# sumansamui/CMOOP_Audio_Processing

Hardware: AMD Instinct MI355X
Metric: candidate-net evals/hour (pop=40, GSC-v2) (higher is better)
Workload: dtype f32

## Files before the change

### cmoop_audio_processing_amd/_lib.py

```python
from __future__ import annotations

import ctypes as C
import os
import re
import subprocess
import threading

_HERE = os.path.dirname(os.path.abspath(__file__))
CSRC = os.path.join(_HERE, "csrc")
LIB_PATH = os.environ.get("CMOOP_LIB_PATH") or os.path.join(CSRC, "libcmoop_hip.so")
HEADER = os.path.join(os.path.dirname(_HERE), "include", "cmoop.h")

_lock = threading.Lock()
_lib = None


class CmoopError(RuntimeError):
    pass


class Config(C.Structure):
    _fields_ = [(n, C.c_int32) for n in (
        "variant", "classes", "epochs", "batch", "patience", "early_stop", "restore_best", "acc_readout",
        "fpr_variant", "shuffle", "eval_batch", "n_slots", "profile_every", "gemm_mode")] + \
# ... 93 lines not shown
    "cmoop_bn_train_fwd": [_V] * 10 + [_I64, _I32, _F64, _F64, _I32, _I32],
    "cmoop_bn_eval_fwd": [_V] * 8 + [_I64, _I32, _F64, _I32],
    "cmoop_bn_bwd": [_V] * 9 + [_I64, _I32, _I32, _I32],
    "cmoop_bn_pool_fwd": [_V] * 5 + [_I32] * 5,
    "cmoop_bn_pool_bwd": [_V] * 10 + [_I32] * 6,
    "cmoop_add_relu": [_V, _V, _V, _I64],
    "cmoop_gap_fwd": [_V, _V, _I32, _I32, _I32],
    "cmoop_gap_bwd": [_V, _V, _V, _I32, _I32, _I32],
    "cmoop_softmax_ce": [_V, _V, _V, _I64, _I64, _I32, _I32, _V, _V, _V],
    "cmoop_softmax_probs": [_V, _V, _I32, _I32],
    "cmoop_adam": [_V, _V, _V, _V, _I64, _F64, _F64, _F64, _F64],
    "cmoop_adam_segments": [_V] * 5 + [_I32] + [_V] * 5 + [_F64] * 4,
    "cmoop_confusion": [_V, _V, _I64, _I32, _I32, _V],
    "cmoop_colsum_small": [_V, _V, _I32, _I32],
    "cmoop_dense_dgrad_small": [_V, _V, _V, _I32, _I32, _I32, _V, _F64],
}


_U32 = C.c_uint32
DENSE_PROTOTYPES = {
    "cmoop_dense_fwd_ex": [_V] * 4 + [_I32] * 5 + [_F64, _U32, _I32, _U32, _V],
    "cmoop_dense_bwd_ex": [_V] * 6 + [_I32] * 4 + [_F64, _I32, _I32],
}

DWCONV_PROTOTYPES = {
    "cmoop_dwconv_fwd": [_V] * 3 + [_I32] * 5,
    "cmoop_dwconv_bwd": [_V] * 5 + [_I32] * 6,
    "cmoop_dwconv_wgrad_slices": [_I32] * 5 + [_V],
    "cmoop_dwconv_time": [_I32] + [_V] * 4 + [_I32] * 6 + [_V],
    "cmoop_plan_dwconvs": [_V, _I32, _I32, _I32, _V, _I32, _V],
# ... 27 lines not shown
                f"{LIB_PATH} is missing: run `python -c 'import __graft_entry__ as g; g.build()'` "
                "(or `make -C cmoop_audio_processing_amd/csrc`). There is no CPU fallback for this path.")
        try:
            L = C.CDLL(LIB_PATH)
        except OSError as e:
            raise CmoopError(f"cannot load {LIB_PATH}: {e}") from e
        L.cmoop_last_error.restype = C.c_char_p
        L.cmoop_abi_version.restype = C.c_int
        for name in declared_symbols():
            fn = getattr(L, name)
            if name not in ("cmoop_last_error", "cmoop_config_default"):
                fn.restype = C.c_int
        L.cmoop_config_default.restype = None
        for name, argtypes in list(STREAM_PROTOTYPES.items()) + list(AUGMENT_PROTOTYPES.items()) + list(PCEN_PROTOTYPES.items()) + \
                list(ELEM_PROTOTYPES.items()) + list(LOSS_PROTOTYPES.items()) + list(DENSE_PROTOTYPES.items()) + list(DWCONV_PROTOTYPES.items()) + \
                list(DISTILL_PROTOTYPES.items()):
            getattr(L, name).argtypes = argtypes
        _lib = L
        return L


def check(rc: int) -> None:
    if rc != 0:
        raise CmoopError(lib().cmoop_last_error().decode("utf-8", "replace"))


def default_config() -> Config:
    c = Config()
    lib().cmoop_config_default(C.byref(c))
    return c

# ... 65 lines not shown
```

### cmoop_audio_processing_amd/csrc/api.hip

```cpp
#include "../../include/cmoop.h"
#include "net.h"

#include <cstring>
#include <memory>
#include <mutex>
#include <vector>

using namespace cmoop;

static thread_local std::string g_err;
static thread_local std::string g_last_kernels;

template <class F>
static int guard(F&& f) {
    try {
        f();
        return 0;
    } catch (const std::exception& e) {
        g_err = e.what();
        return 1;
    } catch (...) {
        g_err = "unknown error";
        return 2;
    }
// ... 881 lines not shown
        h->net->drain_profile();
    });
}
int cmoop_net_get_state(cmoop_net* h, float* params, float* adam_m, float* adam_v, int64_t* iterations, int64_t* steps) {
    return guard([&] {
        long long it = 0, st = 0;
        h->net->get_state(params, adam_m, adam_v, &it, &st);
        if (iterations) *iterations = it;
        if (steps) *steps = st;
    });
}
int cmoop_net_set_state(cmoop_net* h, const float* params, const float* adam_m, const float* adam_v, int64_t iterations,
                        int64_t steps) {
    return guard([&] { h->net->set_state(params, adam_m, adam_v, iterations, steps); });
}
int cmoop_net_set_augment(cmoop_net* h, const cmoop_augment* aug) {
    return guard([&] {
        CMOOP_REQUIRE(h && h->net, "set_augment: NULL net");
        if (!aug) { h->net->set_augment(nullptr); return; }
        const AugmentCfg c = to_augment(aug);
        h->net->set_augment(&c);
    });
}
int cmoop_net_set_loss(cmoop_net* h, const cmoop_loss* loss) {
    return guard([&] {
        CMOOP_REQUIRE(h && h->net, "set_loss: NULL net");
        if (!loss) { h->net->set_loss(nullptr); return; }
        const LossCfg c = to_loss(loss);
        h->net->set_loss(&c);
    });
// ... 461 lines not shown
int cmoop_bn_pool_bwd(const float* g_pooled, const uint8_t* arg, const float* x, const float* mean, const float* invstd,
                      const float* gamma, float* dx, float* dgamma, float* dbeta, float* sums, int32_t B, int32_t H, int32_t W,
                      int32_t C, int32_t mask_x_pos, int32_t blocks) {
    return guard([&] {
        CMOOP_REQUIRE(B >= 1 && H >= 1 && W >= 1, "bn_pool_bwd: empty tensor");
        const int nb = reduce_blocks_arg(blocks, (int64_t)B * H * W, C);
        hipStream_t s = lib_stream();
        Scratch ws(s);
        float* P = ws.floats((size_t)nb * 2 * C + 2 * C);
        launch_bn_pool_bwd_reduce(g_pooled, arg, x, mean, invstd, P, B, H, W, C, nb, s);
        launch_bn_pool_bwd_apply(g_pooled, arg, x, mean, invstd, gamma, P, nb, dx, dgamma, dbeta, B, H, W, C, mask_x_pos, s);
        if (sums) CMOOP_HIP(hipMemcpyAsync(sums, P + (size_t)nb * 2 * C, (size_t)2 * C * 4, hipMemcpyDeviceToDevice, s));
        CMOOP_HIP(hipStreamSynchronize(s));
    });
}
int cmoop_add_relu(const float* a, const float* b, float* y, int64_t n) {
    return guard([&] {
        hipStream_t s = lib_stream();
        launch_add_relu(a, b, y, n, s);
        CMOOP_HIP(hipStreamSynchronize(s));
    });
}
int cmoop_gap_fwd(const float* x, float* y, int32_t B, int32_t HW, int32_t C) {
    return guard([&] {
        CMOOP_REQUIRE(B >= 0 && HW >= 1 && C >= 4, "gap_fwd: HW >= 1, C >= 4");
        hipStream_t s = lib_stream();
        launch_gap_fwd(x, y, B, HW, C, s);
        CMOOP_HIP(hipStreamSynchronize(s));
    });
}
// ... 83 lines not shown
```

### cmoop_audio_processing_amd/csrc/elem.hip

```cpp
#include "kernels.h"
#include <cstdlib>
#include <algorithm>
#include <cmath>
#include <mutex>

namespace cmoop {

typedef float f32x4 __attribute__((ext_vector_type(4)));

__device__ __forceinline__ int64_t gather_row(const int32_t* __restrict__ idx, int64_t pos, int64_t n_rows) {
    int64_t src = idx ? (int64_t)idx[pos] : pos;
    if (n_rows > 0) src = src < 0 ? 0 : (src >= n_rows ? n_rows - 1 : src);
    return src;
}

template <int KS>
__global__ __launch_bounds__(256) void conv1_fwd_kernel(const float* __restrict__ X, const int32_t* __restrict__ idx,
                                                        int64_t row0, const float* __restrict__ Wt,
                                                        const float* __restrict__ bias, float* __restrict__ Y, int B,
                                                        int H, int W, int Cout, int relu, const StepState* __restrict__ st,
                                                        int64_t n_rows) {
    constexpr int TAPS = KS * KS, SEG = 4 + KS - 1, p = (KS - 1) >> 1;
    __shared__ __attribute__((aligned(16))) float Ws[TAPS * 64];
    if (st) row0 = st->row0;
// ... 704 lines not shown
    if (i >= M * K) return;
    const int m = i / K, k = i - m * K;
    float s = 0.f;
    for (int o = 0; o < N; ++o) s = fmaf(dY[(size_t)m * N + o], W[(size_t)o * K + k], s);
    if (mask) s = mask[i] > 0.f ? s * scale : 0.f;
    dX[i] = s;
}

void launch_dense_dgrad_small(const float* dY, const float* W, float* dX, int M, int N, int K, const float* mask,
                              float scale, hipStream_t s) {
    if (M * K == 0) return;
    hipLaunchKernelGGL(dense_dgrad_small_kernel, dim3(cdiv(M * K, 256)), dim3(256), 0, s, dY, W, dX, M, N, K, mask, scale);
    CMOOP_HIP(hipGetLastError());
}

__global__ __launch_bounds__(256) void maxpool_fwd_kernel(const float* __restrict__ X, float* __restrict__ Y,
                                                          uint8_t* __restrict__ arg, int B, int H, int W, int C, int OH,
                                                          int OW) {
    const int C4 = C >> 2;
    const int64_t n = (int64_t)B * OH * OW * C4;
    for (int64_t i = (int64_t)blockIdx.x * 256 + threadIdx.x; i < n; i += (int64_t)gridDim.x * 256) {
        const int c4 = (int)(i % C4);
        int64_t p = i / C4;
        const int ow = (int)(p % OW); p /= OW;
        const int oh = (int)(p % OH);
        const int b = (int)(p / OH);
        f32x4 best;
        uchar4 a = {0, 0, 0, 0};
        bool first = true;
#pragma unroll
        for (int pos = 0; pos < 4; ++pos) {
            const int ih = 2 * oh + (pos >> 1), iw = 2 * ow + (pos & 1);
            if (ih >= H || iw >= W) continue;
            const f32x4 v = *reinterpret_cast<const f32x4*>(X + ((size_t)(b * H + ih) * W + iw) * C + 4 * c4);
            if (first) { best = v; first = false; continue; }
            if (v[0] > best[0]) { best[0] = v[0]; a.x = pos; }
            if (v[1] > best[1]) { best[1] = v[1]; a.y = pos; }
            if (v[2] > best[2]) { best[2] = v[2]; a.z = pos; }
            if (v[3] > best[3]) { best[3] = v[3]; a.w = pos; }
        }
        *reinterpret_cast<f32x4*>(Y + i * 4) = best;
        *reinterpret_cast<uchar4*>(arg + i * 4) = a;
    }
}

void launch_maxpool_fwd(const float* X, float* Y, uint8_t* arg, int B, int H, int W, int C, hipStream_t s) {
    CMOOP_REQUIRE(C % 4 == 0, "maxpool: C % 4");
    const int OH = (H + 1) / 2, OW = (W + 1) / 2;
    const int64_t n = (int64_t)B * OH * OW * (C / 4);
    if (n == 0) return;
    hipLaunchKernelGGL(maxpool_fwd_kernel, dim3(ew_grid(n)), dim3(256), 0, s, X, Y, arg, B, H, W, C, OH, OW);
    CMOOP_HIP(hipGetLastError());
}

__global__ __launch_bounds__(256) void maxpool_bwd_kernel(const float* __restrict__ dY, const uint8_t* __restrict__ arg,
                                                          const float* __restrict__ Y, float* __restrict__ dX, int B,
                                                          int H, int W, int C, int OH, int OW, int mask_y_pos) {
    const int C4 = C >> 2;
    const int64_t n = (int64_t)B * OH * OW * C4;
    for (int64_t i = (int64_t)blockIdx.x * 256 + threadIdx.x; i < n; i += (int64_t)gridDim.x * 256) {
        const int c4 = (int)(i % C4);
        int64_t p = i / C4;
        const int ow = (int)(p % OW); p /= OW;
        const int oh = (int)(p % OH);
        const int b = (int)(p / OH);
        f32x4 g = *reinterpret_cast<const f32x4*>(dY + i * 4);
// ... 14 lines not shown
            *reinterpret_cast<f32x4*>(dX + ((size_t)(b * H + ih) * W + iw) * C + 4 * c4) = o;
        }
    }
}

void launch_maxpool_bwd(const float* dY, const uint8_t* arg, const float* Y, float* dX, int B, int H, int W, int C,
                        int mask_y_pos, hipStream_t s) {
    const int OH = (H + 1) / 2, OW = (W + 1) / 2;
    const int64_t n = (int64_t)B * OH * OW * (C / 4);
    if (n == 0) return;
    hipLaunchKernelGGL(maxpool_bwd_kernel, dim3(ew_grid(n)), dim3(256), 0, s, dY, arg, Y, dX, B, H, W, C, OH, OW,
                       mask_y_pos);
    CMOOP_HIP(hipGetLastError());
}

__global__ __launch_bounds__(256) void bn_pool_fwd_kernel(const float* __restrict__ X, float* __restrict__ Y,
                                                          uint8_t* __restrict__ arg, const float* __restrict__ scale,
                                                          const float* __restrict__ shift, int B, int H, int W, int C,
                                                          int OH, int OW, int relu) {
    const int C4 = C >> 2;
    const int64_t n = (int64_t)B * OH * OW * C4;
    for (int64_t i = (int64_t)blockIdx.x * 256 + threadIdx.x; i < n; i += (int64_t)gridDim.x * 256) {
        const int c4 = (int)(i % C4);
        int64_t p = i / C4;
        const int ow = (int)(p % OW); p /= OW;
        const int oh = (int)(p % OH);
        const int b = (int)(p / OH);
        const f32x4 sc = *reinterpret_cast<const f32x4*>(scale + 4 * c4);
        const f32x4 sh = *reinterpret_cast<const f32x4*>(shift + 4 * c4);
        f32x4 best;
        uchar4 a = {0, 0, 0, 0};
        bool first = true;
#pragma unroll
        for (int pos = 0; pos < 4; ++pos) {
            const int ih = 2 * oh + (pos >> 1), iw = 2 * ow + (pos & 1);
            if (ih >= H || iw >= W) continue;
            const f32x4 x = *reinterpret_cast<const f32x4*>(X + ((size_t)(b * H + ih) * W + iw) * C + 4 * c4);
            f32x4 v;
#pragma unroll
            for (int j = 0; j < 4; ++j) {
                const float t = x[j] * sc[j] + sh[j];
                v[j] = relu ? fmaxf(t, 0.f) : t;
            }
            if (first) { best = v; first = false; continue; }
            if (v[0] > best[0]) { best[0] = v[0]; a.x = pos; }
            if (v[1] > best[1]) { best[1] = v[1]; a.y = pos; }
            if (v[2] > best[2]) { best[2] = v[2]; a.z = pos; }
            if (v[3] > best[3]) { best[3] = v[3]; a.w = pos; }
        }
        *reinterpret_cast<f32x4*>(Y + i * 4) = best;
        *reinterpret_cast<uchar4*>(arg + i * 4) = a;
    }
}

void launch_bn_pool_fwd(const float* X, float* Y, uint8_t* arg, const float* scale, const float* shift, int B, int H, int W,
                        int C, int relu, hipStream_t s) {
    CMOOP_REQUIRE(C % 4 == 0, "bn_pool: C % 4");
    const int OH = (H + 1) / 2, OW = (W + 1) / 2;
    const int64_t n = (int64_t)B * OH * OW * (C / 4);
    if (n == 0) return;
    hipLaunchKernelGGL(bn_pool_fwd_kernel, dim3(ew_grid(n)), dim3(256), 0, s, X, Y, arg, scale, shift, B, H, W, C, OH, OW, relu);
    CMOOP_HIP(hipGetLastError());
}

struct PooledGrad {
    const float* g; const uint8_t* arg;
    int H, W, OH, OW, C;
    __device__ __forceinline__ f32x4 at(int64_t row, int c) const {
        const int iw = (int)(row % W);
        const int64_t t = row / W;
        const int ih = (int)(t % H), b = (int)(t / H);
        const size_t o = (((size_t)b * OH + (ih >> 1)) * OW + (iw >> 1)) * C + c;
        const f32x4 gv = *reinterpret_cast<const f32x4*>(g + o);
        const uchar4 a = *reinterpret_cast<const uchar4*>(arg + o);
        const int pos = ((ih & 1) << 1) | (iw & 1);
        return f32x4{a.x == pos ? gv[0] : 0.f, a.y == pos ? gv[1] : 0.f, a.z == pos ? gv[2] : 0.f, a.w == pos ? gv[3] : 0.f};
// ... 1033 lines not shown
```

### cmoop_audio_processing_amd/csrc/kernels.h

```cpp
#pragma once
#include "common.h"
#include <string>
#include <vector>

namespace cmoop {

struct ConvGeom {
    int B, H, W, Cin;
    int OH, OW, Cout;
    int KH, KW, stride;
    int pad_t, pad_l;
    int M() const { return B * OH * OW; }
    int K() const { return KH * KW * Cin; }
};
inline ConvGeom conv_geometry(int B, int H, int W, int Cin, int Cout, int KS, int stride) {
    ConvGeom g;
    g.B = B; g.H = H; g.W = W; g.Cin = Cin; g.Cout = Cout; g.KH = g.KW = KS; g.stride = stride;
    g.OH = (H + stride - 1) / stride; g.OW = (W + stride - 1) / stride;
    const int th = (g.OH - 1) * stride + KS - H, tw = (g.OW - 1) * stride + KS - W;
    g.pad_t = (th > 0 ? th : 0) / 2; g.pad_l = (tw > 0 ? tw : 0) / 2;
    return g;
}

enum GemmMode { GEMM_DEFAULT = -1, GEMM_FP32 = 0, GEMM_FP32_DMA = 1 , GEMM_BF16X3 = 2, GEMM_BF16 = 3,
// ... 177 lines not shown
void launch_bn_finalize(const float* P, int blocks, int64_t M, int C, const float* gamma, const float* beta,
                        float* moving_mean, float* moving_var, float* mean, float* invstd, float* scale,
                        float* shift, float eps, float momentum, float one_minus_momentum, hipStream_t s);
void launch_bn_eval_prepare(const float* gamma, const float* beta, const float* moving_mean,
                            const float* moving_var, float* scale, float* shift, int C, float eps, hipStream_t s);
void launch_scale_shift(const float* X, float* Y, const float* scale, const float* shift, int64_t M, int C,
                        int relu, hipStream_t s);
void launch_bn_bwd_apply(const float* dY, const float* X, const float* mean, const float* invstd,
                         const float* gamma, const float* P, int blocks, float* dX, float* dgamma, float* dbeta,
                         int64_t M, int C, int mask_x_pos, hipStream_t s);
void launch_colsum_small(const float* X, float* out, int M, int C, hipStream_t s);
void launch_dense_dgrad_small(const float* dY, const float* W, float* dX, int M, int N, int K, const float* mask,
                              float scale, hipStream_t s);
void launch_colsum_finalize(const float* P, int blocks, int C, float* out, hipStream_t s);

void launch_maxpool_fwd(const float* X, float* Y, uint8_t* arg, int B, int H, int W, int C, hipStream_t s);
void launch_maxpool_bwd(const float* dY, const uint8_t* arg, const float* Y, float* dX, int B, int H, int W, int C,
                        int mask_y_pos, hipStream_t s);
void launch_bn_pool_fwd(const float* X, float* Y, uint8_t* arg, const float* scale, const float* shift, int B, int H, int W,
                        int C, int relu, hipStream_t s);
void launch_bn_pool_bwd_reduce(const float* g_pooled, const uint8_t* arg, const float* X, const float* mean, const float* invstd,
                               float* P, int B, int H, int W, int C, int blocks, hipStream_t s);
void launch_bn_pool_bwd_apply(const float* g_pooled, const uint8_t* arg, const float* X, const float* mean, const float* invstd,
                              const float* gamma, const float* P, int blocks, float* dX, float* dgamma, float* dbeta, int B,
                              int H, int W, int C, int mask_x_pos, hipStream_t s);
void launch_add_relu(const float* A, const float* Bt, float* Y, int64_t n, hipStream_t s);
void launch_gap_fwd(const float* X, float* Y, int B, int HW, int C, hipStream_t s);
void launch_gap_bwd(const float* dY, const float* X, float* dX, int B, int HW, int C, hipStream_t s);
void launch_softmax_ce(const float* Z, const int32_t* labels, const int32_t* idx, int64_t row0, int B, int C,
                       float* dZ, double* acc, int32_t* preds, hipStream_t s, const StepState* st = nullptr, int64_t n_rows = 0);
void launch_softmax_probs(const float* Z, float* P, int B, int C, hipStream_t s);
void launch_window_gather(const float* feat, float* chunk, int64_t w0, int B, int hop, int T, int F, int db, int db_ref_max,
                          float amin, float top_db, const double* mean, const double* scale, hipStream_t s);
void launch_adam(float* w, const float* g, float* m, float* v, int64_t n, float alpha, float c1, float c2,
                 float eps, hipStream_t s, const StepState* st = nullptr, const float* alpha_table = nullptr);
// ... 65 lines not shown
```

### cmoop_audio_processing_amd/csrc/net.h

```cpp
#pragma once
#include "kernels.h"
#include <atomic>
#include <functional>
#include <map>
#include <mutex>
#include <set>
#include <string>
#include <vector>

namespace cmoop {

struct NetConfig {
    int variant = 0, classes = 10, epochs = 300, batch = 64, patience = 5;
    int early_stop = 1, restore_best = 0, acc_readout = 0, fpr_variant = 0, shuffle = 1;
    int eval_batch = 256, n_slots = 8, profile_every = 0;
    int gemm_mode = GEMM_FP32;
    double lr = 1e-3, beta1 = 0.9, beta2 = 0.999, adam_eps = 1e-7, bn_eps = 1e-3, bn_momentum = 0.99, dropout = 0.3;
};

struct DropoutParams {
    uint32_t thr;
    float keep_scale;
    static uint32_t stream(int layer) { return STREAM_DROPOUT + (uint32_t)layer; }
};
// ... 97 lines not shown
    int rowtab_rows = 0;
    void* rowtab_d = nullptr;
    int rowtab_d_rows = 0;
    int64_t w_off = 0, b_off = 0, wd_off = -1;
    int64_t slab_off = -1;
    size_t slab_floats = 0;
    int tensor_index = 0;
    int64_t gamma_off = 0, beta_off = 0, mm_off = 0, mv_off = 0;
    int relu_after = 0, mask_in_pos = 0;
    int fuse_pool = 0;
    int feeds_bn = 0;
    float* bn_buf = nullptr;
    uint8_t* arg = nullptr;
    int mask_y_pos = 0;
    int fused_into_bn = 0;
};

struct NetPlan {
    std::vector<Act> acts;
    std::vector<Op> ops;
    int logits = -1;
    int64_t n_params = 0;
    size_t splitk_floats(int batch, int Bmax) const;
    std::string launch_plan(int batch, int Bmax, int B, bool train) const;
};
NetPlan plan_net(const int32_t gene[6], const NetConfig& cfg, int T, int F);

class Net : public GemmHook {
  public:
    const GemmTiming* begin(int cls, double flops) override;
// ... 19 lines not shown
    void run_epoch(const float* X, const int32_t* y, int64_t n_train, int epoch, int32_t* idx_scratch);

    void train_step(const float* X, const int32_t* y, const int32_t* idx, int64_t row0, int B);
    void train_step_targets(const float* x_rows, const float* t, const float* w, const int32_t* primary, int B);
    void train_step_distill_targets(const float* x_rows, const float* t, const float* w, const int32_t* primary, const float* q,
                                    double alpha, double temperature, int B);
    void begin_fit(int64_t total_steps);
    void begin_epoch();
    void train_step_stateful(const float* X, const int32_t* y, const int32_t* idx, int B);
    void evaluate(const float* X, const int32_t* y, int64_t n, double* loss_sum, long long* correct, int32_t* preds);
    void predict(const float* X, int64_t n, float* probs);
    void predict_logits(const float* X, int64_t n, float* logits);
    void predict_stream(const float* feat, int64_t n_frames, int hop, bool db_scale, bool db_ref_max, float db_amin, float top_db,
                        const double* mean, const double* scale, float* probs);
    void read_train_metrics(double* loss_sum, long long* correct, bool reset);
    void drain_profile();
    hipStream_t stream() const { return stream_; }
    uint32_t seed() const { return seed_; }
    const NetConfig& config() const { return cfg_; }
    int feature_T() const { return T_; }
    int feature_F() const { return F_; }
    long long steps_done() const { return step_; }
    long long iterations_done() const { return iterations_; }

  private:
    void build_plan();
    void forward(const float* X, const int32_t* idx, int64_t row0, int B, bool train, const StepState* st = nullptr);
    void backward(const float* X, const int32_t* idx, int64_t row0, int B, const StepState* st = nullptr);
    void step_body(const float* X, const int32_t* y, const int32_t* idx, int64_t row0, int B, const StepState* st);
    void optimiser_step(int B, const StepState* st);
    ConvBuffers buffers_of(const Op& op) const;
    float* dalloc(size_t floats);

    int32_t gene_[6];
    NetConfig cfg_;
    int T_, F_, Bmax_;
    uint32_t seed_;
    hipStream_t stream_;
    std::vector<Act> acts_;
    std::vector<Op> ops_;
    std::vector<void*> allocs_;
    int64_t n_params_ = 0;
// ... 63 lines not shown
```

### cmoop_audio_processing_amd/csrc/net.hip

```cpp
#include "net.h"

#include <algorithm>
#include <chrono>
#include <cmath>
#include <cstdlib>
#include <cstring>
#include <functional>
#include <map>
#include <numeric>
#include <thread>

namespace cmoop {

static const int FC_LADDER[5][4] = {{0, 0, 0, 0}, {64, 0, 0, 0}, {128, 64, 0, 0}, {256, 128, 64, 0}, {512, 256, 128, 64}};

void validate_gene(const int32_t g[6]) {
    const bool ok = (g[0] == 16 || g[0] == 32 || g[0] == 64) && (g[1] == 3 || g[1] == 5) && (g[2] == 0 || g[2] == 1) &&
                    (g[3] >= 1 && g[3] <= 3) && (g[4] >= 1 && g[4] <= 4) && (g[5] == 0 || g[5] == 1);
    CMOOP_REQUIRE(ok, "gene outside the search space (filters{16,32,64}, kernel{3,5}, bn{0,1}, res{1..3}, fc{1..4}, dropout{0,1})");
}

DropoutParams dropout_params(double rate) {
    CMOOP_REQUIRE(rate >= 0.0 && rate < 1.0, "dropout must be in [0,1)");
    return DropoutParams{(uint32_t)(rate * 16777216.0), (float)(1.0 / (1.0 - rate))};
// ... 259 lines not shown
        const int skip = add_conv(OP_CONV, x, 2 * c, 1, 2, 0, in_relu, 1.f, 1);
        int y;
        if (A) {
            y = add_sepconv(x, 2 * c, k, !bn, in_relu);
            if (bn) y = add_bn(y, 1, 0);
            y = add_sepconv(y, 2 * c, k, 0, 1);
            if (bn) y = add_bn(y, 0, 0);
            y = add_pool(y, 0);
        } else {
            y = add_sepconv(x, 2 * c, k, 1, in_relu);
            if (bn) y = add_bn(y, 0, 1);
            y = add_pool(y, !bn);
        }
        Op op; op.kind = OP_ADDRELU; op.in = y; op.in2 = skip;
        op.out = new_act(acts[y].H, acts[y].W, acts[y].C);
        ops.push_back(op);
        x = op.out;
        c *= 2;
    }
    {
        Op op; op.kind = OP_GAP; op.in = x;
        op.out = new_act(1, 1, acts[x].C);
        ops.push_back(op);
        x = op.out;
    }
    const float keep_scale = dropout_params(cfg.dropout).keep_scale;
    for (int i = 0; i < fc; ++i) {
        const int in_relu = i > 0;
        const float ms = (in_relu && dr) ? keep_scale : 1.f;
        x = add_conv(OP_DENSE, x, FC_LADDER[fc][i], 1, 1, 1, in_relu, ms, 0);
// ... 402 lines not shown
        case OP_BN: {
            const Act& ia = acts_[op.in];
            const int64_t M = (int64_t)B * ia.H * ia.W;
            const int C = op.Cout;
            float *mean = op.bn_buf, *invstd = mean + C, *scale = invstd + C, *shift = scale + C;
            if (train) {
                int nb = fused_stats_blocks_;
                fused_stats_blocks_ = 0;
                if (nb == 0) {
                    nb = colreduce_blocks(M, C);
                    launch_colstats(ia.data, red_ws_, M, C, nb, stream_);
                }
                launch_bn_finalize(red_ws_, nb, M, C, params_ + op.gamma_off, params_ + op.beta_off, params_ + op.mm_off,
                                   params_ + op.mv_off, mean, invstd, scale, shift, (float)cfg_.bn_eps, (float)cfg_.bn_momentum,
                                   (float)(1.0 - cfg_.bn_momentum), stream_);
            } else {
                launch_bn_eval_prepare(params_ + op.gamma_off, params_ + op.beta_off, params_ + op.mm_off,
                                       params_ + op.mv_off, scale, shift, C, (float)cfg_.bn_eps, stream_);
            }
            if (op.fuse_pool) {
                const Op& pool = ops_[oi + 1];
                launch_bn_pool_fwd(ia.data, acts_[pool.out].data, pool.arg, scale, shift, B, ia.H, ia.W, C, op.relu_after, stream_);
            } else {
                launch_scale_shift(ia.data, acts_[op.out].data, scale, shift, M, C, op.relu_after, stream_);
            }
            break;
        }
        case OP_POOL: {
            if (op.fused_into_bn) break;
            const Act& ia = acts_[op.in];
            launch_maxpool_fwd(ia.data, acts_[op.out].data, op.arg, B, ia.H, ia.W, ia.C, stream_);
            break;
        }
        case OP_ADDRELU:
            launch_add_relu(acts_[op.in].data, acts_[op.in2].data, acts_[op.out].data,
                            (int64_t)B * acts_[op.out].per_sample(), stream_);
            break;
        case OP_GAP: {
            const Act& ia = acts_[op.in];
            launch_gap_fwd(ia.data, acts_[op.out].data, B, ia.H * ia.W, ia.C, stream_);
            break;
        }
        }
    }
}

void Net::backward(const float* X, const int32_t* idx, int64_t row0, int B, const StepState* st) {
    slab_segs_.clear();
    launch_flip_transpose_all(params_, wd_ws_, flip_table_, flip_layers_, flip_max_elems_, stream_);
    for (int oi = (int)ops_.size() - 1; oi >= 0; --oi) {
        const Op& op = ops_[oi];
        switch (op.kind) {
        case OP_DENSE: {
            const float* dY = acts_[op.out].grad;
            Act& ia = acts_[op.in];
            const char* du = std::getenv("CMOOP_DENSE_UNFUSED");
            const bool unfused = du && du[0] == '1';
            if (!unfused) {
                launch_dense_bwd(ia.data, dY, params_ + op.w_off, grads_ + op.w_off, grads_ + op.b_off, ia.grad, B, op.Cout, op.Cin,
// ... 41 lines not shown
            if (op.fuse_pool) {
                const Op& pool = ops_[oi + 1];
                launch_bn_pool_bwd_reduce(acts_[pool.out].grad, pool.arg, ia.data, mean, invstd, red_ws_, B, ia.H, ia.W, C, nb, stream_);
                launch_bn_pool_bwd_apply(acts_[pool.out].grad, pool.arg, ia.data, mean, invstd, params_ + op.gamma_off, red_ws_, nb,
                                         ia.grad, grads_ + op.gamma_off, grads_ + op.beta_off, B, ia.H, ia.W, C, op.mask_in_pos, stream_);
                break;
            }
            launch_bn_bwd_reduce(acts_[op.out].grad, ia.data, mean, invstd, red_ws_, M, C, nb, stream_);
            launch_bn_bwd_apply(acts_[op.out].grad, ia.data, mean, invstd, params_ + op.gamma_off, red_ws_, nb, ia.grad,
                                grads_ + op.gamma_off, grads_ + op.beta_off, M, C, op.mask_in_pos, stream_);
            break;
        }
        case OP_POOL: {
            if (op.fused_into_bn) break;
            const Act& ia = acts_[op.in];
            launch_maxpool_bwd(acts_[op.out].grad, op.arg, acts_[op.out].data, ia.grad, B, ia.H, ia.W, ia.C, op.mask_y_pos,
                               stream_);
            break;
        }
        case OP_ADDRELU:
            break;
        case OP_GAP: {
            const Act& ia = acts_[op.in];
            launch_gap_bwd(acts_[op.out].grad, ia.data, ia.grad, B, ia.H * ia.W, ia.C, stream_);
            break;
        }
        case OP_CONV1: {
            if (batch_in_)
                launch_conv1_wgrad(batch_in_, nullptr, 0, acts_[op.out].grad, wgrad_ws_ + op.slab_off, B, T_, F_, op.Cout, op.KS, stream_,
                                   nullptr, 0);
// ... 141 lines not shown
    std::vector<float> tab(total_steps);
    const double b1 = cfg_.beta1, b2 = cfg_.beta2;
    for (int64_t i = 0; i < total_steps; ++i) {
        const double t = (double)(i + 1);
        tab[i] = (float)(cfg_.lr * std::sqrt(1.0 - std::pow(b2, t)) / (1.0 - std::pow(b1, t)));
    }
    alpha_tab_ = dalloc(total_steps);
    alpha_tab_n_ = total_steps;
    if (!st_dev_) st_dev_ = reinterpret_cast<StepState*>(dalloc(8));
    CMOOP_HIP(hipMemcpyAsync(alpha_tab_, tab.data(), total_steps * 4, hipMemcpyHostToDevice, stream_));
    const StepState st0{0, (unsigned)step_, (unsigned)iterations_};
    CMOOP_HIP(hipMemcpyAsync(st_dev_, &st0, sizeof(StepState), hipMemcpyHostToDevice, stream_));
    CMOOP_HIP(hipStreamSynchronize(stream_));
    static const bool use_graph = [] { const char* v = std::getenv("CMOOP_GRAPH"); return v && v[0] == '1'; }();
    if (!use_graph) graph_ok_ = false;
}

void Net::begin_epoch() {
    host_row0_ = 0;
    if (st_dev_) CMOOP_HIP(hipMemsetAsync(&st_dev_->row0, 0, sizeof(long long), stream_));
}

void Net::train_step_stateful(const float* X, const int32_t* y, const int32_t* idx, int B) {
    CMOOP_REQUIRE(B >= 1 && B <= cfg_.batch, "train batch larger than configured");
    if (!st_dev_) {
        train_step(X, y, idx, host_row0_, B);
        host_row0_ += B;
        return;
    }
    CMOOP_REQUIRE(iterations_ < alpha_tab_n_, "train_step_stateful outside begin_fit's step budget");
// ... 164 lines not shown
        }
        idx = idx_scratch;
    }
    if (st_dev_) {
        const StepState st0{0, (unsigned)step_, (unsigned)iterations_};
        CMOOP_HIP(hipMemcpyAsync(st_dev_, &st0, sizeof(StepState), hipMemcpyHostToDevice, stream_));
        CMOOP_HIP(hipStreamSynchronize(stream_));
    }
    begin_epoch();
    for (int64_t s = 0; s < n_train; s += cfg_.batch)
        train_step_stateful(X, y, idx, (int)std::min<int64_t>(cfg_.batch, n_train - s));
}

void Net::evaluate(const float* X, const int32_t* y, int64_t n, double* loss_sum, long long* correct, int32_t* preds) {
    CMOOP_HIP(hipMemsetAsync(acc_eval_, 0, 16, stream_));
    for (int64_t s = 0; s < n; s += cfg_.eval_batch) {
        const int B = (int)std::min<int64_t>(cfg_.eval_batch, n - s);
        forward(X, nullptr, s, B, false);
        launch_softmax_ce(acts_[logits_].data, y, nullptr, s, B, cfg_.classes, nullptr, acc_eval_, preds ? preds + s : nullptr,
                          stream_);
    }
    double host[2];
    CMOOP_HIP(hipMemcpyAsync(host, acc_eval_, 16, hipMemcpyDeviceToHost, stream_));
    CMOOP_HIP(hipStreamSynchronize(stream_));
    *loss_sum = host[0];
    std::memcpy(correct, &host[1], 8);
}

void Net::predict(const float* X, int64_t n, float* probs) {
    CMOOP_REQUIRE(n >= 0 && (n == 0 || (X && probs)), "predict: NULL buffer");
    for (int64_t s = 0; s < n; s += cfg_.eval_batch) {
        const int B = (int)std::min<int64_t>(cfg_.eval_batch, n - s);
        forward(X, nullptr, s, B, false);
        launch_softmax_probs(acts_[logits_].data, probs + s * cfg_.classes, B, cfg_.classes, stream_);
    }
    CMOOP_HIP(hipStreamSynchronize(stream_));
}

void Net::predict_logits(const float* X, int64_t n, float* logits) {
    CMOOP_REQUIRE(n >= 0 && (n == 0 || (X && logits)), "predict_logits: NULL buffer");
    for (int64_t s = 0; s < n; s += cfg_.eval_batch) {
        const int B = (int)std::min<int64_t>(cfg_.eval_batch, n - s);
        forward(X, nullptr, s, B, false);
        CMOOP_HIP(hipMemcpyAsync(logits + s * cfg_.classes, acts_[logits_].data, (size_t)B * cfg_.classes * 4, hipMemcpyDeviceToDevice,
                                 stream_));
    }
    CMOOP_HIP(hipStreamSynchronize(stream_));
}

int64_t stream_windows(int64_t n_frames, int T, int hop) {
    CMOOP_REQUIRE(hop >= 1, "stream windows: hop_frames must be at least 1");
    CMOOP_REQUIRE(T >= 1 && n_frames >= T, "stream windows: the stream has " + std::to_string(n_frames) + " frames, a window needs " + std::to_string(T));
    return 1 + (n_frames - T) / hop;
}

void Net::predict_stream(const float* feat, int64_t n_frames, int hop, bool db_scale, bool db_ref_max, float db_amin, float top_db,
                         const double* mean, const double* scale, float* probs) {
    const int64_t n = stream_windows(n_frames, T_, hop);
    CMOOP_REQUIRE(feat && probs, "predict_stream: NULL buffer");
    CMOOP_REQUIRE((mean == nullptr) == (scale == nullptr), "predict_stream: mean and scale come together (both or neither)");
    const int B0 = (int)std::min<int64_t>(cfg_.eval_batch, n);
    float* chunk = static_cast<float*>(pool_alloc((size_t)B0 * T_ * F_ * 4));
    double* ms = mean ? static_cast<double*>(pool_alloc((size_t)2 * F_ * 8)) : nullptr;
    auto cleanup = [&]() { hipStreamSynchronize(stream_); pool_free(chunk); if (ms) pool_free(ms); };
    try {
        if (ms) {
            CMOOP_HIP(hipMemcpyAsync(ms, mean, (size_t)F_ * 8, hipMemcpyHostToDevice, stream_));
            CMOOP_HIP(hipMemcpyAsync(ms + F_, scale, (size_t)F_ * 8, hipMemcpyHostToDevice, stream_));
        }
        for (int64_t w = 0; w < n; w += cfg_.eval_batch) {
            const int B = (int)std::min<int64_t>(cfg_.eval_batch, n - w);
            launch_window_gather(feat, chunk, w, B, hop, T_, F_, db_scale ? 1 : 0, db_ref_max ? 1 : 0, db_amin, top_db, ms,
                                 ms ? ms + F_ : nullptr, stream_);
            forward(chunk, nullptr, 0, B, false);
            launch_softmax_probs(acts_[logits_].data, probs + w * cfg_.classes, B, cfg_.classes, stream_);
        }
    } catch (...) {
        cleanup();
        throw;
    }
    cleanup();
}

void Net::read_train_metrics(double* loss_sum, long long* correct, bool reset) {
// ... 198 lines not shown
```

### cmoop_audio_processing_amd/session.py

```python
from __future__ import annotations

import ctypes as C

import numpy as np

from . import _lib, genes as G
from .evaluator import EvalConfig


FROM_CONFIG = object()


class NetSession:
    def __init__(self, gene, config: EvalConfig, T: int, F: int, seed: int):
        self.gene = tuple(int(v) for v in gene)
        G.validate_gene(self.gene)
        self.config = config
        self._h = C.c_void_p()
        g = (C.c_int32 * 6)(*self.gene)
        cfg = config.to_struct()
        _lib.check(_lib.lib().cmoop_net_create(g, C.byref(cfg), C.c_int32(T), C.c_int32(F), C.c_uint32(seed & 0xFFFFFFFF),
                                               C.byref(self._h)))
        n = C.c_int64()
        _lib.check(_lib.lib().cmoop_net_total_params(self._h, C.byref(n)))
# ... 185 lines not shown
                                                       _lib.ptr(probs)))
        return probs

    def get_state(self):
        p, m, v = (np.empty(self.n_params, np.float32) for _ in range(3))
        it, st = C.c_int64(), C.c_int64()
        _lib.check(_lib.lib().cmoop_net_get_state(self._h, _lib.ptr(p), _lib.ptr(m), _lib.ptr(v), C.byref(it), C.byref(st)))
        return {"params": p, "m": m, "v": v, "iterations": int(it.value), "steps": int(st.value)}

    def set_state(self, state) -> None:
        p, m, v = (np.ascontiguousarray(state[k], np.float32) for k in ("params", "m", "v"))
        assert p.size == m.size == v.size == self.n_params
        _lib.check(_lib.lib().cmoop_net_set_state(self._h, _lib.ptr(p), _lib.ptr(m), _lib.ptr(v),
                                                  C.c_int64(int(state["iterations"])), C.c_int64(int(state["steps"]))))

    def set_gather_rows(self, n_rows: int) -> None:
        _lib.check(_lib.lib().cmoop_net_set_gather_rows(self._h, C.c_int64(int(n_rows))))

    def run_epoch(self, X, y, epoch: int) -> None:
        self._require_teacher()
        import torch
        torch.cuda.synchronize()
        _lib.check(_lib.lib().cmoop_net_run_epoch(self._h, _lib.ptr(X), _lib.ptr(y), C.c_int64(len(X)), C.c_int32(int(epoch))))

    def fit(self, X_train, y_train, X_val, y_val):
        self._require_teacher()
        import torch
        torch.cuda.synchronize()
        d = _lib.DatasetStruct()
        d.x_train, d.y_train, d.n_train = X_train.data_ptr(), y_train.data_ptr(), len(X_train)
# ... 23 lines not shown
```

### include/cmoop.h

```cpp
#ifndef CMOOP_H
#define CMOOP_H

#include <stdint.h>

#ifdef __cplusplus
extern "C" {
#endif

#define CMOOP_ABI_VERSION 3

#define CMOOP_VARIANT_A 0
#define CMOOP_VARIANT_B 1
#define CMOOP_VARIANT_A_DS 2
#define CMOOP_VARIANT_B_DS 3

#define CMOOP_FPR_V1 0
#define CMOOP_FPR_V1_QUIRK 1
#define CMOOP_FPR_V3 2

#define CMOOP_GEMM_DEFAULT 0
#define CMOOP_GEMM_FP32 1
#define CMOOP_GEMM_BF16X3 2
#define CMOOP_GEMM_BF16 3

// ... 192 lines not shown
                             float* probs_dev);
int cmoop_net_get_state(cmoop_net* net, float* params, float* adam_m, float* adam_v, int64_t* iterations, int64_t* steps);
int cmoop_net_set_state(cmoop_net* net, const float* params, const float* adam_m, const float* adam_v, int64_t iterations,
                        int64_t steps);
int cmoop_net_set_augment(cmoop_net* net, const cmoop_augment* aug );
int cmoop_net_set_loss(cmoop_net* net, const cmoop_loss* loss );
int cmoop_net_train_step_targets(cmoop_net* net, const float* x_rows_dev, const float* t_dev, const float* w_dev,
                                 const int32_t* primary_dev, int32_t B);
int cmoop_net_loss_buffers(cmoop_net* net, int64_t out[4]);
int cmoop_net_set_distill(cmoop_net* net, const cmoop_distill* distill );
int cmoop_net_train_step_distill_targets(cmoop_net* net, const float* x_rows_dev, const float* t_dev, const float* w_dev,
                                         const int32_t* primary_dev, const float* q_dev, double alpha, double temperature, int32_t B);
int cmoop_net_predict_logits(cmoop_net* net, const float* x_dev , int64_t n, float* logits_dev );
int cmoop_net_set_gather_rows(cmoop_net* net, int64_t n_rows);
int cmoop_net_run_epoch(cmoop_net* net, const float* x_train_dev, const int32_t* y_train_dev, int64_t n_train, int32_t epoch);
int cmoop_net_fit(cmoop_net* net, const cmoop_dataset* ds, int32_t hist_cap, double* val_loss_hist, double* val_acc_hist,
                  int32_t* epochs_run, int32_t* best_epoch, double* acc, double* fpr, double* val_loss);
int cmoop_epoch_permutation(uint32_t seed, uint32_t epoch, int64_t n, int32_t* out_host);
int cmoop_epoch_permutation_device(uint32_t seed, uint32_t epoch, int64_t n, int32_t* out_dev);

int cmoop_conv_fwd(const float* x_dev, const float* w_dev, const float* bias_dev, float* y_dev, int32_t B, int32_t H,
                   int32_t W, int32_t Cin, int32_t Cout, int32_t KS, int32_t stride, int32_t relu);
int cmoop_conv_bwd(const float* x_dev, const float* w_dev, const float* dy_dev, float* dx_dev, float* dw_dev, float* db_dev,
                   int32_t B, int32_t H, int32_t W, int32_t Cin, int32_t Cout, int32_t KS, int32_t stride, int32_t mask_relu);
int cmoop_conv_fwd_trainer(const float* x_dev, const float* w_dev, const float* bias_dev, float* y_dev, int32_t B, int32_t H,
                           int32_t W, int32_t Cin, int32_t Cout, int32_t KS, int32_t stride, int32_t relu, double* col_sum,
                           double* col_sumsq, int32_t* stats_fused);
int cmoop_conv_bwd_trainer(const float* x_dev, const float* w_dev, const float* dy_dev, float* dx_dev, float* dw_dev,
                           float* db_dev, int32_t B, int32_t H, int32_t W, int32_t Cin, int32_t Cout, int32_t KS, int32_t stride,
                           int32_t mask_relu);
// ... 19 lines not shown
                      int32_t W, int32_t C, int32_t mask_y_pos);
int cmoop_bn_train_fwd(const float* x_dev, const float* gamma_dev, const float* beta_dev, float* moving_mean_dev,
                       float* moving_var_dev, float* y_dev, float* mean_dev, float* invstd_dev, float* scale_dev, float* shift_dev,
                       int64_t M, int32_t C, double eps, double momentum, int32_t relu, int32_t blocks);
int cmoop_bn_eval_fwd(const float* x_dev, const float* gamma_dev, const float* beta_dev, const float* moving_mean_dev,
                      const float* moving_var_dev, float* y_dev, float* scale_dev, float* shift_dev, int64_t M, int32_t C,
                      double eps, int32_t relu);
int cmoop_bn_bwd(const float* dy_dev, const float* x_dev, const float* mean_dev, const float* invstd_dev, const float* gamma_dev,
                 float* dx_dev, float* dgamma_dev, float* dbeta_dev, float* sums_dev, int64_t M, int32_t C, int32_t mask_x_pos,
                 int32_t blocks);
int cmoop_bn_pool_fwd(const float* x_dev, const float* scale_dev, const float* shift_dev, float* y_dev, uint8_t* arg_dev, int32_t B,
                      int32_t H, int32_t W, int32_t C, int32_t relu);
int cmoop_bn_pool_bwd(const float* g_pooled_dev, const uint8_t* arg_dev, const float* x_dev, const float* mean_dev,
                      const float* invstd_dev, const float* gamma_dev, float* dx_dev, float* dgamma_dev, float* dbeta_dev,
                      float* sums_dev, int32_t B, int32_t H, int32_t W, int32_t C, int32_t mask_x_pos, int32_t blocks);
int cmoop_add_relu(const float* a_dev, const float* b_dev, float* y_dev, int64_t n);
int cmoop_gap_fwd(const float* x_dev, float* y_dev, int32_t B, int32_t HW, int32_t C);
int cmoop_gap_bwd(const float* dy_dev, const float* x_dev, float* dx_dev, int32_t B, int32_t HW, int32_t C);
int cmoop_softmax_ce(const float* z_dev, const int32_t* labels_dev, const int32_t* idx_dev, int64_t row0, int64_t n_rows, int32_t B,
                     int32_t C, float* dz_dev, double* acc_dev, int32_t* preds_dev);
int cmoop_softmax_probs(const float* z_dev, float* p_dev, int32_t B, int32_t C);
int cmoop_adam(float* w_dev, const float* g_dev, float* m_dev, float* v_dev, int64_t n, double alpha, double beta1, double beta2,
               double eps);
int cmoop_adam_segments(float* w_dev, float* g_dev, float* m_dev, float* v_dev, const float* slab_dev, int32_t count,
                        const int64_t* off, const int64_t* n, const int32_t* S, const int64_t* stride, const int64_t* slab_off,
                        double alpha, double beta1, double beta2, double eps);
int cmoop_confusion(const int32_t* y_true_dev, const int32_t* y_pred_dev, int64_t n, int32_t C, int32_t force_true_zero,
                    int64_t* cm_dev);
int cmoop_colsum_small(const float* x_dev, float* out_dev, int32_t M, int32_t C);
int cmoop_dense_dgrad_small(const float* dy_dev, const float* w_dev, float* dx_dev, int32_t M, int32_t N, int32_t K,
// ... 8 lines not shown
```

Baseline: 440.1.

## Fuse residual add+ReLU into maxpool epilogue and hoist eval BN prepare

Residual-block tails where a maxpool feeds an add+ReLU now run as one kernel: the pool (or BN+pool) kernel adds the skip tensor and applies ReLU before writing, and the pooled intermediate becomes virtual (never materialised). This removes one elementwise launch plus a full write and read of the pooled activation per block. Separately, eval-mode BN scale/shift preparation moves out of every forward batch into a once-per-call prepare_inference. The fusion applies only when the pool does not mask backward by its output. The backward pass still reads the pool's output gradient, which carries a risk if the virtual buffer is referenced.

Result: no change. 441.1 (median of 6 runs) (+0.2%).

```diff
diff --git a/cmoop_audio_processing_amd/_lib.py b/cmoop_audio_processing_amd/_lib.py
--- a/cmoop_audio_processing_amd/_lib.py
+++ b/cmoop_audio_processing_amd/_lib.py
@@ -131,6 +131,13 @@
     "cmoop_confusion": [_V, _V, _I64, _I32, _I32, _V],
     "cmoop_colsum_small": [_V, _V, _I32, _I32],
     "cmoop_dense_dgrad_small": [_V, _V, _V, _I32, _I32, _I32, _V, _F64],
+}
+
+
+TAIL_PROTOTYPES = {
+    "cmoop_pool_add_relu_fwd": [_V] * 4 + [_I32] * 4,
+    "cmoop_bn_pool_add_relu_fwd": [_V] * 6 + [_I32] * 5,
+    "cmoop_net_plan_summary": [_V, _V],
 }
 
 
@@ -188,7 +195,7 @@
         L.cmoop_config_default.restype = None
         for name, argtypes in list(STREAM_PROTOTYPES.items()) + list(AUGMENT_PROTOTYPES.items()) + list(PCEN_PROTOTYPES.items()) + \
                 list(ELEM_PROTOTYPES.items()) + list(LOSS_PROTOTYPES.items()) + list(DENSE_PROTOTYPES.items()) + list(DWCONV_PROTOTYPES.items()) + \
-                list(DISTILL_PROTOTYPES.items()):
+                list(DISTILL_PROTOTYPES.items()) + list(TAIL_PROTOTYPES.items()):
             getattr(L, name).argtypes = argtypes
         _lib = L
         return L
diff --git a/cmoop_audio_processing_amd/csrc/api.hip b/cmoop_audio_processing_amd/csrc/api.hip
--- a/cmoop_audio_processing_amd/csrc/api.hip
+++ b/cmoop_audio_processing_amd/csrc/api.hip
@@ -919,6 +919,14 @@
                         int64_t steps) {
     return guard([&] { h->net->set_state(params, adam_m, adam_v, iterations, steps); });
 }
+int cmoop_net_plan_summary(cmoop_net* h, int64_t out[3]) {
+    return guard([&] {
+        CMOOP_REQUIRE(h && h->net && out, "plan_summary: NULL net or output");
+        long long v[3];
+        h->net->plan_summary(v);
+        for (int i = 0; i < 3; ++i) out[i] = v[i];
+    });
+}
 int cmoop_net_set_augment(cmoop_net* h, const cmoop_augment* aug) {
     return guard([&] {
         CMOOP_REQUIRE(h && h->net, "set_augment: NULL net");
@@ -1410,6 +1418,23 @@
         CMOOP_HIP(hipStreamSynchronize(s));
     });
 }
+int cmoop_pool_add_relu_fwd(const float* x, const float* skip, float* y, uint8_t* arg, int32_t B, int32_t H, int32_t W, int32_t C) {
+    return guard([&] {
+        CMOOP_REQUIRE(skip != nullptr, "pool_add_relu_fwd: NULL skip operand");
+        hipStream_t s = lib_stream();
+        launch_maxpool_fwd(x, y, arg, B, H, W, C, s, skip);
+        CMOOP_HIP(hipStreamSynchronize(s));
+    });
+}
+int cmoop_bn_pool_add_relu_fwd(const float* x, const float* scale, const float* shift, const float* skip, float* y, uint8_t* arg,
+                               int32_t B, int32_t H, int32_t W, int32_t C, int32_t relu) {
+    return guard([&] {
+        CMOOP_REQUIRE(skip != nullptr, "bn_pool_add_relu_fwd: NULL skip operand");
+        hipStream_t s = lib_stream();
+        launch_bn_pool_fwd(x, y, arg, scale, shift, B, H, W, C, relu, s, skip);
+        CMOOP_HIP(hipStreamSynchronize(s));
+    });
+}
 int cmoop_add_relu(const float* a, const float* b, float* y, int64_t n) {
     return guard([&] {
         hipStream_t s = lib_stream();
diff --git a/cmoop_audio_processing_amd/csrc/elem.hip b/cmoop_audio_processing_amd/csrc/elem.hip
--- a/cmoop_audio_processing_amd/csrc/elem.hip
+++ b/cmoop_audio_processing_amd/csrc/elem.hip
@@ -742,9 +742,10 @@
     CMOOP_HIP(hipGetLastError());
 }
 
-__global__ __launch_bounds__(256) void maxpool_fwd_kernel(const float* __restrict__ X, float* __restrict__ Y,
-                                                          uint8_t* __restrict__ arg, int B, int H, int W, int C, int OH,
-                                                          int OW) {
+template <bool SKIP>
+__device__ __forceinline__ void maxpool_fwd_body(const float* __restrict__ X, const float* __restrict__ skip,
+                                                 float* __restrict__ Y, uint8_t* __restrict__ arg, int B, int H, int W, int C,
+                                                 int OH, int OW) {
     const int C4 = C >> 2;
     const int64_t n = (int64_t)B * OH * OW * C4;
     for (int64_t i = (int64_t)blockIdx.x * 256 + threadIdx.x; i < n; i += (int64_t)gridDim.x * 256) {
@@ -767,17 +768,35 @@
             if (v[2] > best[2]) { best[2] = v[2]; a.z = pos; }
             if (v[3] > best[3]) { best[3] = v[3]; a.w = pos; }
         }
+        if constexpr (SKIP) {
+            const f32x4 sk = *reinterpret_cast<const f32x4*>(skip + i * 4);
+#pragma unroll
+            for (int j = 0; j < 4; ++j) best[j] = fmaxf(best[j] + sk[j], 0.f);
+        }
         *reinterpret_cast<f32x4*>(Y + i * 4) = best;
         *reinterpret_cast<uchar4*>(arg + i * 4) = a;
     }
 }
 
-void launch_maxpool_fwd(const float* X, float* Y, uint8_t* arg, int B, int H, int W, int C, hipStream_t s) {
+__global__ __launch_bounds__(256) void maxpool_fwd_kernel(const float* __restrict__ X, float* __restrict__ Y,
+                                                          uint8_t* __restrict__ arg, int B, int H, int W, int C, int OH,
+                                                          int OW) {
+    maxpool_fwd_body<false>(X, nullptr, Y, arg, B, H, W, C, OH, OW);
+}
+
+__global__ __launch_bounds__(256) void pool_add_relu_fwd_kernel(const float* __restrict__ X, const float* __restrict__ skip,
+                                                                float* __restrict__ Y, uint8_t* __restrict__ arg, int B, int H,
+                                                                int W, int C, int OH, int OW) {
+    maxpool_fwd_body<true>(X, skip, Y, arg, B, H, W, C, OH, OW);
+}
+
+void launch_maxpool_fwd(const float* X, float* Y, uint8_t* arg, int B, int H, int W, int C, hipStream_t s, const float* skip) {
     CMOOP_REQUIRE(C % 4 == 0, "maxpool: C % 4");
     const int OH = (H + 1) / 2, OW = (W + 1) / 2;
     const int64_t n = (int64_t)B * OH * OW * (C / 4);
     if (n == 0) return;
-    hipLaunchKernelGGL(maxpool_fwd_kernel, dim3(ew_grid(n)), dim3(256), 0, s, X, Y, arg, B, H, W, C, OH, OW);
+    if (skip) hipLaunchKernelGGL(pool_add_relu_fwd_kernel, dim3(ew_grid(n)), dim3(256), 0, s, X, skip, Y, arg, B, H, W, C, OH, OW);
+    else hipLaunchKernelGGL(maxpool_fwd_kernel, dim3(ew_grid(n)), dim3(256), 0, s, X, Y, arg, B, H, W, C, OH, OW);
     CMOOP_HIP(hipGetLastError());
 }
 
@@ -822,10 +841,11 @@
     CMOOP_HIP(hipGetLastError());
 }
 
-__global__ __launch_bounds__(256) void bn_pool_fwd_kernel(const float* __restrict__ X, float* __restrict__ Y,
-                                                          uint8_t* __restrict__ arg, const float* __restrict__ scale,
-                                                          const float* __restrict__ shift, int B, int H, int W, int C,
-                                                          int OH, int OW, int relu) {
+template <bool SKIP>
+__device__ __forceinline__ void bn_pool_fwd_body(const float* __restrict__ X, const float* __restrict__ skip,
+                                                 float* __restrict__ Y, uint8_t* __restrict__ arg,
+                                                 const float* __restrict__ scale, const float* __restrict__ shift, int B, int H,
+                                                 int W, int C, int OH, int OW, int relu) {
     const int C4 = C >> 2;
     const int64_t n = (int64_t)B * OH * OW * C4;
     for (int64_t i = (int64_t)blockIdx.x * 256 + threadIdx.x; i < n; i += (int64_t)gridDim.x * 256) {
@@ -856,18 +876,42 @@
             if (v[2] > best[2]) { best[2] = v[2]; a.z = pos; }
             if (v[3] > best[3]) { best[3] = v[3]; a.w = pos; }
         }
+        if constexpr (SKIP) {
+            const f32x4 sk = *reinterpret_cast<const f32x4*>(skip + i * 4);
+#pragma unroll
+            for (int j = 0; j < 4; ++j) best[j] = fmaxf(best[j] + sk[j], 0.f);
+        }
         *reinterpret_cast<f32x4*>(Y + i * 4) = best;
         *reinterpret_cast<uchar4*>(arg + i * 4) = a;
     }
 }
 
+__global__ __launch_bounds__(256) void bn_pool_fwd_kernel(const float* __restrict__ X, float* __restrict__ Y,
+                                                          uint8_t* __restrict__ arg, const float* __restrict__ scale,
+                                                          const float* __restrict__ shift, int B, int H, int W, int C,
+                                                          int OH, int OW, int relu) {
+    bn_pool_fwd_body<false>(X, nullptr, Y, arg, scale, shift, B, H, W, C, OH, OW, relu);
+}
+
+__global__ __launch_bounds__(256) void bn_pool_add_relu_fwd_kernel(const float* __restrict__ X, const float* __restrict__ skip,
+                                                                   float* __restrict__ Y, uint8_t* __restrict__ arg,
+                                                                   const float* __restrict__ scale,
+                                                                   const float* __restrict__ shift, int B, int H, int W, int C,
+                                                                   int OH, int OW, int relu) {
+    bn_pool_fwd_body<true>(X, skip, Y, arg, scale, shift, B, H, W, C, OH, OW, relu);
+}
+
 void launch_bn_pool_fwd(const float* X, float* Y, uint8_t* arg, const float* scale, const float* shift, int B, int H, int W,
-                        int C, int relu, hipStream_t s) {
+                        int C, int relu, hipStream_t s, const float* skip) {
     CMOOP_REQUIRE(C % 4 == 0, "bn_pool: C % 4");
     const int OH = (H + 1) / 2, OW = (W + 1) / 2;
     const int64_t n = (int64_t)B * OH * OW * (C / 4);
     if (n == 0) return;
-    hipLaunchKernelGGL(bn_pool_fwd_kernel, dim3(ew_grid(n)), dim3(256), 0, s, X, Y, arg, scale, shift, B, H, W, C, OH, OW, relu);
+    if (skip)
+        hipLaunchKernelGGL(bn_pool_add_relu_fwd_kernel, dim3(ew_grid(n)), dim3(256), 0, s, X, skip, Y, arg, scale, shift, B, H, W, C,
+                           OH, OW, relu);
+    else
+        hipLaunchKernelGGL(bn_pool_fwd_kernel, dim3(ew_grid(n)), dim3(256), 0, s, X, Y, arg, scale, shift, B, H, W, C, OH, OW, relu);
     CMOOP_HIP(hipGetLastError());
 }
 
diff --git a/cmoop_audio_processing_amd/csrc/kernels.h b/cmoop_audio_processing_amd/csrc/kernels.h
--- a/cmoop_audio_processing_amd/csrc/kernels.h
+++ b/cmoop_audio_processing_amd/csrc/kernels.h
@@ -215,11 +215,12 @@
                               float scale, hipStream_t s);
 void launch_colsum_finalize(const float* P, int blocks, int C, float* out, hipStream_t s);
 
-void launch_maxpool_fwd(const float* X, float* Y, uint8_t* arg, int B, int H, int W, int C, hipStream_t s);
+void launch_maxpool_fwd(const float* X, float* Y, uint8_t* arg, int B, int H, int W, int C, hipStream_t s,
+                        const float* skip = nullptr);
 void launch_maxpool_bwd(const float* dY, const uint8_t* arg, const float* Y, float* dX, int B, int H, int W, int C,
                         int mask_y_pos, hipStream_t s);
 void launch_bn_pool_fwd(const float* X, float* Y, uint8_t* arg, const float* scale, const float* shift, int B, int H, int W,
-                        int C, int relu, hipStream_t s);
+                        int C, int relu, hipStream_t s, const float* skip = nullptr);
 void launch_bn_pool_bwd_reduce(const float* g_pooled, const uint8_t* arg, const float* X, const float* mean, const float* invstd,
                                float* P, int B, int H, int W, int C, int blocks, hipStream_t s);
 void launch_bn_pool_bwd_apply(const float* g_pooled, const uint8_t* arg, const float* X, const float* mean, const float* invstd,
diff --git a/cmoop_audio_processing_amd/csrc/net.h b/cmoop_audio_processing_amd/csrc/net.h
--- a/cmoop_audio_processing_amd/csrc/net.h
+++ b/cmoop_audio_processing_amd/csrc/net.h
@@ -135,6 +135,8 @@
     uint8_t* arg = nullptr;
     int mask_y_pos = 0;
     int fused_into_bn = 0;
+    int tail_skip = -1, tail_out = -1;
+    int fused_into_pool = 0;
 };
 
 struct NetPlan {
@@ -184,6 +186,7 @@
     void predict_stream(const float* feat, int64_t n_frames, int hop, bool db_scale, bool db_ref_max, float db_amin, float top_db,
                         const double* mean, const double* scale, float* probs);
     void read_train_metrics(double* loss_sum, long long* correct, bool reset);
+    void plan_summary(long long out[3]) const;
     void drain_profile();
     hipStream_t stream() const { return stream_; }
     uint32_t seed() const { return seed_; }
@@ -196,6 +199,7 @@
   private:
     void build_plan();
     void forward(const float* X, const int32_t* idx, int64_t row0, int B, bool train, const StepState* st = nullptr);
+    void prepare_inference();
     void backward(const float* X, const int32_t* idx, int64_t row0, int B, const StepState* st = nullptr);
     void step_body(const float* X, const int32_t* y, const int32_t* idx, int64_t row0, int B, const StepState* st);
     void optimiser_step(int B, const StepState* st);
diff --git a/cmoop_audio_processing_amd/csrc/net.hip b/cmoop_audio_processing_amd/csrc/net.hip
--- a/cmoop_audio_processing_amd/csrc/net.hip
+++ b/cmoop_audio_processing_amd/csrc/net.hip
@@ -297,6 +297,14 @@
         }
         Op op; op.kind = OP_ADDRELU; op.in = y; op.in2 = skip;
         op.out = new_act(acts[y].H, acts[y].W, acts[y].C);
+        const char* unf = std::getenv("CMOOP_TAIL_UNFUSED");
+        Op& pool = ops.back();
+        if (!(unf && unf[0] == '1') && pool.kind == OP_POOL && pool.out == y && !pool.mask_y_pos) {
+            pool.tail_skip = skip;
+            pool.tail_out = op.out;
+            op.fused_into_pool = 1;
+            acts[y].virt = true;
+        }
         ops.push_back(op);
         x = op.out;
         c *= 2;
@@ -729,13 +737,12 @@
                 launch_bn_finalize(red_ws_, nb, M, C, params_ + op.gamma_off, params_ + op.beta_off, params_ + op.mm_off,
                                    params_ + op.mv_off, mean, invstd, scale, shift, (float)cfg_.bn_eps, (float)cfg_.bn_momentum,
                                    (float)(1.0 - cfg_.bn_momentum), stream_);
-            } else {
-                launch_bn_eval_prepare(params_ + op.gamma_off, params_ + op.beta_off, params_ + op.mm_off,
-                                       params_ + op.mv_off, scale, shift, C, (float)cfg_.bn_eps, stream_);
             }
             if (op.fuse_pool) {
                 const Op& pool = ops_[oi + 1];
-                launch_bn_pool_fwd(ia.data, acts_[pool.out].data, pool.arg, scale, shift, B, ia.H, ia.W, C, op.relu_after, stream_);
+                const bool tail = pool.tail_out >= 0;
+                launch_bn_pool_fwd(ia.data, acts_[tail ? pool.tail_out : pool.out].data, pool.arg, scale, shift, B, ia.H, ia.W, C,
+                                   op.relu_after, stream_, tail ? acts_[pool.tail_skip].data : nullptr);
             } else {
                 launch_scale_shift(ia.data, acts_[op.out].data, scale, shift, M, C, op.relu_after, stream_);
             }
@@ -744,10 +751,13 @@
         case OP_POOL: {
             if (op.fused_into_bn) break;
             const Act& ia = acts_[op.in];
-            launch_maxpool_fwd(ia.data, acts_[op.out].data, op.arg, B, ia.H, ia.W, ia.C, stream_);
+            const bool tail = op.tail_out >= 0;
+            launch_maxpool_fwd(ia.data, acts_[tail ? op.tail_out : op.out].data, op.arg, B, ia.H, ia.W, ia.C, stream_,
+                               tail ? acts_[op.tail_skip].data : nullptr);
             break;
         }
         case OP_ADDRELU:
+            if (op.fused_into_pool) break;
             launch_add_relu(acts_[op.in].data, acts_[op.in2].data, acts_[op.out].data,
                             (int64_t)B * acts_[op.out].per_sample(), stream_);
             break;
@@ -758,6 +768,15 @@
         }
         }
     }
+}
+
+void Net::prepare_inference() {
+    for (const Op& op : ops_)
+        if (op.kind == OP_BN) {
+            float *scale = op.bn_buf + 2 * op.Cout, *shift = scale + op.Cout;
+            launch_bn_eval_prepare(params_ + op.gamma_off, params_ + op.beta_off, params_ + op.mm_off, params_ + op.mv_off, scale,
+                                   shift, op.Cout, (float)cfg_.bn_eps, stream_);
+        }
 }
 
 void Net::backward(const float* X, const int32_t* idx, int64_t row0, int B, const StepState* st) {
@@ -829,6 +848,7 @@
         case OP_POOL: {
             if (op.fused_into_bn) break;
             const Act& ia = acts_[op.in];
+            CMOOP_REQUIRE(!op.mask_y_pos || acts_[op.out].data, "pool backward masks by a pooled tensor that was never materialised");
             launch_maxpool_bwd(acts_[op.out].grad, op.arg, acts_[op.out].data, ia.grad, B, ia.H, ia.W, ia.C, op.mask_y_pos,
                                stream_);
             break;
@@ -1000,6 +1020,14 @@
     CMOOP_HIP(hipStreamSynchronize(stream_));
     static const bool use_graph = [] { const char* v = std::getenv("CMOOP_GRAPH"); return v && v[0] == '1'; }();
     if (!use_graph) graph_ok_ = false;
+}
+
+void Net::plan_summary(long long out[3]) const {
+    out[0] = out[1] = out[2] = 0;
+    for (const Op& op : ops_)
+        if (op.kind == OP_ADDRELU) { ++out[0]; out[1] += op.fused_into_pool; }
+    for (size_t i = 1; i < acts_.size(); ++i)
+        if (!acts_[i].virt) out[2] += (long long)Bmax_ * (long long)acts_[i].per_sample() * 4;
 }
 
 void Net::begin_epoch() {
@@ -1194,6 +1222,7 @@
 
 void Net::evaluate(const float* X, const int32_t* y, int64_t n, double* loss_sum, long long* correct, int32_t* preds) {
     CMOOP_HIP(hipMemsetAsync(acc_eval_, 0, 16, stream_));
+    prepare_inference();
     for (int64_t s = 0; s < n; s += cfg_.eval_batch) {
         const int B = (int)std::min<int64_t>(cfg_.eval_batch, n - s);
         forward(X, nullptr, s, B, false);
@@ -1209,6 +1238,7 @@
 
 void Net::predict(const float* X, int64_t n, float* probs) {
     CMOOP_REQUIRE(n >= 0 && (n == 0 || (X && probs)), "predict: NULL buffer");
+    prepare_inference();
     for (int64_t s = 0; s < n; s += cfg_.eval_batch) {
         const int B = (int)std::min<int64_t>(cfg_.eval_batch, n - s);
         forward(X, nullptr, s, B, false);
@@ -1219,6 +1249,7 @@
 
 void Net::predict_logits(const float* X, int64_t n, float* logits) {
     CMOOP_REQUIRE(n >= 0 && (n == 0 || (X && logits)), "predict_logits: NULL buffer");
+    prepare_inference();
     for (int64_t s = 0; s < n; s += cfg_.eval_batch) {
         const int B = (int)std::min<int64_t>(cfg_.eval_batch, n - s);
         forward(X, nullptr, s, B, false);
@@ -1248,6 +1279,7 @@
             CMOOP_HIP(hipMemcpyAsync(ms, mean, (size_t)F_ * 8, hipMemcpyHostToDevice, stream_));
             CMOOP_HIP(hipMemcpyAsync(ms + F_, scale, (size_t)F_ * 8, hipMemcpyHostToDevice, stream_));
         }
+        prepare_inference();
         for (int64_t w = 0; w < n; w += cfg_.eval_batch) {
             const int B = (int)std::min<int64_t>(cfg_.eval_batch, n - w);
             launch_window_gather(feat, chunk, w, B, hop, T_, F_, db_scale ? 1 : 0, db_ref_max ? 1 : 0, db_amin, top_db, ms,
diff --git a/cmoop_audio_processing_amd/session.py b/cmoop_audio_processing_amd/session.py
--- a/cmoop_audio_processing_amd/session.py
+++ b/cmoop_audio_processing_amd/session.py
@@ -223,6 +223,11 @@
         _lib.check(_lib.lib().cmoop_net_set_state(self._h, _lib.ptr(p), _lib.ptr(m), _lib.ptr(v),
                                                   C.c_int64(int(state["iterations"])), C.c_int64(int(state["steps"]))))
 
+    def plan_summary(self):
+        out = (C.c_int64 * 3)()
+        _lib.check(_lib.lib().cmoop_net_plan_summary(self._h, out))
+        return dict(zip(("blocks", "fused_tails", "activation_bytes"), (int(v) for v in out)))
+
     def set_gather_rows(self, n_rows: int) -> None:
         _lib.check(_lib.lib().cmoop_net_set_gather_rows(self._h, C.c_int64(int(n_rows))))
 
diff --git a/include/cmoop.h b/include/cmoop.h
--- a/include/cmoop.h
+++ b/include/cmoop.h
@@ -230,6 +230,7 @@
 int cmoop_net_predict_logits(cmoop_net* net, const float* x_dev , int64_t n, float* logits_dev );
 int cmoop_net_set_gather_rows(cmoop_net* net, int64_t n_rows);
 int cmoop_net_run_epoch(cmoop_net* net, const float* x_train_dev, const int32_t* y_train_dev, int64_t n_train, int32_t epoch);
+int cmoop_net_plan_summary(cmoop_net* net, int64_t out[3]);
 int cmoop_net_fit(cmoop_net* net, const cmoop_dataset* ds, int32_t hist_cap, double* val_loss_hist, double* val_acc_hist,
                   int32_t* epochs_run, int32_t* best_epoch, double* acc, double* fpr, double* val_loss);
 int cmoop_epoch_permutation(uint32_t seed, uint32_t epoch, int64_t n, int32_t* out_host);
@@ -279,6 +280,10 @@
 int cmoop_bn_pool_bwd(const float* g_pooled_dev, const uint8_t* arg_dev, const float* x_dev, const float* mean_dev,
                       const float* invstd_dev, const float* gamma_dev, float* dx_dev, float* dgamma_dev, float* dbeta_dev,
                       float* sums_dev, int32_t B, int32_t H, int32_t W, int32_t C, int32_t mask_x_pos, int32_t blocks);
+int cmoop_pool_add_relu_fwd(const float* x_dev, const float* skip_dev, float* y_dev, uint8_t* arg_dev, int32_t B, int32_t H,
+                            int32_t W, int32_t C);
+int cmoop_bn_pool_add_relu_fwd(const float* x_dev, const float* scale_dev, const float* shift_dev, const float* skip_dev,
+                               float* y_dev, uint8_t* arg_dev, int32_t B, int32_t H, int32_t W, int32_t C, int32_t relu);
 int cmoop_add_relu(const float* a_dev, const float* b_dev, float* y_dev, int64_t n);
 int cmoop_gap_fwd(const float* x_dev, float* y_dev, int32_t B, int32_t HW, int32_t C);
 int cmoop_gap_bwd(const float* dy_dev, const float* x_dev, float* dx_dev, int32_t B, int32_t HW, int32_t C);
```
